# nosnoc/LCQPow

Hardware: AMD Instinct MI355X
Metric: LCQPs/sec (batched dense n=256,nC=512,nComp=64) (higher is better)
Workload: dtype f64; 1 GPU; synthetic dense batch=1024/GPU n=256 nC=512 nComp=64 (BASELINE configs[2]; SplitMix64 seed0=0x4C43515000000001, perturbStep=0, printLevel=NONE); global_batch=1024, parallelism=batch-sharded x1, no collective, solved=1024

## Files before the change

lcqpow_amd/csrc/lcqp_dev.hpp:

```cpp
#pragma once
#include "lcqp_wg.hpp"
#include "../../include/lcqp_hip.h"

namespace lcqp {

enum { V_G, V_GPHI, V_GTIL, V_XK, V_PK, V_XNEW, V_GK, V_QX, V_CX, V_QP, V_CP, V_STATK, V_TMP,
       V_XQ, V_XA, V_XT, V_R1, V_C, V_DU, V_W, V_RHS, V_LB, V_UB, V_X0, V_R1S, V_GS, V_ATY, V_QXN, V_XS, V_XREF, V_NUM };
enum { M_L, M_U, M_RHOV, M_YQ, M_YA, M_ZA, M_YT, M_EX, M_COEF, M_EXS, M_DY, M_RN, M_MG, M_YLV, M_HOTV, M_NUM };
enum { I_ST, I_STT, I_DEP, I_PRIO, I_SLOT, I_LIST, I_LIST2, I_HOTC, I_NUM };
enum { S_R2, S_DY, S_D0, S_SV, S_W, S_NUM };

struct InstInfo {
    int mE, nfin, hasY0, setupFail, haveSolution, isSetup, nT, prioCtr;
    int ndep, ns;
    int cNnz, kReady, rnReady, nHot;
    double scale, sigma, spv, rhoAdmm, phiConst;
    int warm, pad0;
    double rho0;
    double hist[64];
    double work[6];
};

struct DevBatch {
    int B, n, np, nC, nComp, mA, boxcap, mEcap, capS, nblk, nd;
// ... 19 lines not shown
};

template <int NCH>
struct Ctx {
    static constexpr int np = 128 * NCH;
    const DevBatch* db;
    int b, n, nC, nComp, mA, mE, capS, nblk;
    double *Q, *C, *E, *Et, *F1, *FK, *S, *S2, *DS, *D1, *dscr, *MM;
    double *nv, *mv, *sv;
    int *mi, *idx, *boxidx, *crow;
    InstInfo* info;
    Lds lds;
    int cAdmm, cTrials, cFact, cCorr, cSweeps;
#ifdef LCQP_PROFILE
    unsigned long long prof[16], tlast;
#endif

    __device__ __forceinline__ double* V(int k) const { return nv + (size_t)k * np; }
    __device__ __forceinline__ double* M(int k) const { return mv + (size_t)k * db->mEcap; }
    __device__ __forceinline__ int* I(int k) const { return mi + (size_t)k * db->mEcap; }
    __device__ __forceinline__ double* Sv(int k) const { return sv + (size_t)k * db->capS; }
};

template <int NCH>
__device__ __forceinline__ Ctx<NCH> make_ctx(const DevBatch& db, int b, Lds lds)
{
    Ctx<NCH> c;
    constexpr int np = 128 * NCH;
    c.db = &db; c.b = b; c.n = db.n; c.nC = db.nC; c.nComp = db.nComp; c.mA = db.mA; c.capS = db.capS; c.nblk = db.nblk;
    c.Q = db.Q + (size_t)b * np * np; c.C = db.C + (size_t)b * np * np;
    c.E = db.E + (size_t)b * db.mEcap * np; c.Et = db.Et + (size_t)b * db.mEcap * np;
    c.F1 = db.F1 + (size_t)b * np * np; c.FK = db.FK + (size_t)b * np * np;
    c.S = db.S + (size_t)b * db.capS * db.capS;
    c.MM = db.MM + (size_t)b * db.mMld * db.mMld;
    c.S2 = db.S2 + (size_t)b * db.capS * db.capS; c.DS = db.DS + (size_t)b * (db.capS / 64) * 4096;
    c.crow = db.crow + (size_t)b * db.capS;
    c.D1 = db.D1 + (size_t)b * db.nblk * 4096; c.dscr = db.dscr + (size_t)b * 4096;
    c.nv = db.nv + (size_t)b * V_NUM * np; c.mv = db.mv + (size_t)b * M_NUM * db.mEcap;
    c.sv = db.sv + (size_t)b * S_NUM * db.capS;
    c.mi = db.mi + (size_t)b * I_NUM * db.mEcap; c.idx = db.idx + (size_t)b * db.capS;
    c.boxidx = db.boxidx + (size_t)b * np;
    c.info = db.info + b;
    c.mE = uniform_i(c.info->mE);
    c.lds = lds;
    c.cAdmm = c.cTrials = c.cFact = c.cCorr = c.cSweeps = 0;
#ifdef LCQP_PROFILE
    for (int k = 0; k < 16; k++) c.prof[k] = 0;
    c.tlast = clock64();
#endif
    return c;
}

enum { P_LCQP = 0, P_RESID = 1, P_GRAM = 2, P_CHOL = 3, P_CORR_L1 = 4, P_CORR_ROWS = 5, P_CORR_S = 6, P_ADMM = 7, P_MISC = 8, P_DEL = 9, P_UPD_PRE = 10 };
#if defined(LCQP_PROFILE) && !defined(LCQP_PROFILE_BULK)
#define PROF(c, k) do { unsigned long long t_ = clock64(); (c).prof[k] += t_ - (c).tlast; (c).tlast = t_; } while (0)
#else
#define PROF(c, k) do { } while (0)
#endif
#if defined(LCQP_PROFILE) && defined(LCQP_PROFILE_BULK)
#define PROFB0(c) do { (c).tlast = clock64(); } while (0)
#define PROFB(c, k) do { unsigned long long t_ = clock64(); (c).prof[k] += t_ - (c).tlast; (c).tlast = t_; } while (0)
#else
#define PROFB0(c) do { } while (0)
#define PROFB(c, k) do { } while (0)
#endif

__device__ __forceinline__ double clipd(double v, double lo, double hi) { return v < lo ? lo : (v > hi ? hi : v); }

template <int NCH>
__device__ __forceinline__ void qp_admm(Ctx<NCH>& c, const double* g, int n_it)
{
    constexpr int np = 128 * NCH;
    const lcqp_options_t& o = c.db->opt;
    const int t = tid_here(), mE = c.mE;
    const double alpha = o.admmAlpha, sigma = c.info->sigma;
    double *xa = c.V(V_XA), *rhs = c.V(V_RHS), *w = c.V(V_W);
    double *ya = c.M(M_YA), *za = c.M(M_ZA), *rhov = c.M(M_RHOV), *coef = c.M(M_COEF), *ex = c.M(M_EX), *dyl = c.M(M_DY);
    const double *l = c.M(M_L), *u = c.M(M_U);
    PROF(c, P_MISC);
    for (int it = 0; it < n_it; it++) {
        const int t = tid_here();
        for (int r = t; r < mE; r += WG) coef[r] = rhov[r] * za[r] - ya[r];
        __syncthreads();
        wg_rows<NCH>(c.E, nullptr, mE, nullptr, nullptr, coef, c.lds,
                     [&](int i, double s) { rhs[i] = sigma * xa[i] - g[i] + s; });
        wg_trsv<wg_ncopy(NCH) == 2>(c.FK, np, c.nblk, rhs, true, c.lds);
        wg_trsv<wg_ncopy(NCH) == 2>(c.FK, np, c.nblk, rhs, false, c.lds);
        wg_rows<NCH>(c.E, nullptr, mE, rhs, ex, nullptr, c.lds, [](int, double) {});
        const bool last = (it == n_it - 1);
        for (int r = t; r < mE; r += WG) {
            const double zr = alpha * ex[r] + (1.0 - alpha) * za[r];
            const double rv = rhov[r];
            const double yold = ya[r];
            double yn;
            if (rv > 0.0) {
                const double zn = clipd(zr + yold / rv, l[r], u[r]);
                yn = yold + rv * (zr - zn);
                za[r] = zn;
            } else {
                za[r] = zr;
                yn = 0.0;
            }
            ya[r] = yn;
            if (last) dyl[r] = yn - yold;
        }
        for (int i = t; i < np; i += WG) {
            const double xold = xa[i], xn = alpha * rhs[i] + (1.0 - alpha) * xold;
            xa[i] = xn;
            if (last) w[i] = xn - xold;
        }
// ... 160 lines not shown
constexpr int TI_FAST_CHUNKS = 4;

template <int NCH>
__device__ __forceinline__ void ti_reset(Ctx<NCH>& c, int& nT, int& ns)
{
    int* rslot = c.I(I_SLOT);
    for (int r = tid_here(); r < c.mE; r += WG) rslot[r] = -1;
    for (int a = tid_here(); a < c.capS; a += WG) c.idx[a] = -1;
    nT = 0; ns = 0;
    __syncthreads();
}

template <int NK, int D>
__device__ __forceinline__ void ti_apply_fast(const double* __restrict__ Ti, int ld, const double* tv, double* out, int nT, int ns, double* red, const int* crow, const int* slotRow)
{
    const int l = lane_id(), w = wave_id(), t = tid_here();
    double tr[NK], acc[NK];
    int first[NK];
#pragma unroll
    for (int k = 0; k < NK; k++) {
        const int sl = 64 * k + l; tr[k] = (sl < ns) ? tv[sl] : 0.0; acc[k] = 0.0;
        first[k] = (sl < ns && slotRow[sl] >= 0) ? crow[sl] : (1 << 30);
    }
    for (int j0 = w; j0 < nT; j0 += NWAVE * D) {
        double rv[D][NK];
#pragma unroll
        for (int d = 0; d < D; d++) {
            const int j = j0 + NWAVE * d;
#pragma unroll
            for (int k = 0; k < NK; k++) {
                const int sl = 64 * k + l;
                rv[d][k] = (j < nT && j >= first[k]) ? Ti[(size_t)j * ld + sl] : 0.0;
            }
        }
#pragma unroll
        for (int d = 0; d < D; d++) {
            double dsum = 0.0;
#pragma unroll
            for (int k = 0; k < NK; k++) dsum += rv[d][k] * tr[k];
            const double u = wave_sum(dsum);
#pragma unroll
            for (int k = 0; k < NK; k++) acc[k] += rv[d][k] * u;
        }
    }
    __syncthreads();
#pragma unroll
    for (int k = 0; k < NK; k++) red[w * 256 + 64 * k + l] = acc[k];
    __syncthreads();
    for (int sl = t; sl < 64 * NK; sl += WG) out[sl] = (sl < ns) ? (red[sl] + red[256 + sl]) + (red[512 + sl] + red[768 + sl]) : 0.0;
    __syncthreads();
}

template <int NCH>
__device__ __forceinline__ void ti_apply(Ctx<NCH>& c, const double* tv, double* out, int nT, int ns)
{
    const int ld = c.capS, l = lane_id(), w = wave_id(), t = tid_here();
    const int nk = (ns + 63) >> 6;
    const double* Ti = c.S;
    if (nk <= TI_FAST_CHUNKS) {
        double* red = c.lds.arena;
        if (nk <= 1) ti_apply_fast<1, 16>(Ti, ld, tv, out, nT, ns, red, c.crow, c.idx);
        else if (nk == 2) ti_apply_fast<2, 8>(Ti, ld, tv, out, nT, ns, red, c.crow, c.idx);
        else if (nk == 3) ti_apply_fast<3, 6>(Ti, ld, tv, out, nT, ns, red, c.crow, c.idx);
        else ti_apply_fast<4, 4>(Ti, ld, tv, out, nT, ns, red, c.crow, c.idx);
    } else {
        constexpr int MAXK = (max_active(NCH) + 63) / 64;
        double* ts = c.lds.arena;
        double* us = c.lds.arena + 64 * nk;
        for (int sl = t; sl < 64 * nk; sl += WG) ts[sl] = (sl < ns) ? tv[sl] : 0.0;
        __syncthreads();
        for (int j = w; j < nT; j += NWAVE) {
            double dsum = 0.0;
#pragma unroll 4
            for (int k = 0; k < nk; k++) { const int sl = 64 * k + l; dsum += (sl < ns ? Ti[(size_t)j * ld + sl] : 0.0) * ts[sl]; }
            dsum = wave_sum(dsum);
            if (l == 0) us[j] = dsum;
        }
        __syncthreads();
        double acc[MAXK];
#pragma unroll
        for (int k = 0; k < MAXK; k++) acc[k] = 0.0;
        for (int j = w; j < nT; j += NWAVE) {
            const double u = us[j];
#pragma unroll
            for (int k = 0; k < MAXK; k++) { const int sl = 64 * k + l; if (k < nk && sl < ns) acc[k] += Ti[(size_t)j * ld + sl] * u; }
        }
        __syncthreads();
        double* red = c.lds.arena;
#pragma unroll
        for (int k = 0; k < MAXK; k++) if (k < nk) red[w * 64 * nk + 64 * k + l] = acc[k];
        __syncthreads();
        for (int sl = t; sl < 64 * nk; sl += WG)
            out[sl] = (sl < ns) ? (red[sl] + red[64 * nk + sl]) + (red[2 * 64 * nk + sl] + red[3 * 64 * nk + sl]) : 0.0;
        __syncthreads();
    }
}

template <int NCH>
__device__ __forceinline__ int ti_bulk(Ctx<NCH>& c, int na, double tau, int& nT, int& ns)
{
    const int ld = c.capS, t = tid_here(), mMld = c.db->mMld;
    const int nb = (na + 63) >> 6, nn = 64 * nb;
    int *idx = c.idx, *rslot = c.I(I_SLOT), *dep = c.I(I_DEP);
    double *F = c.S2, *Ti = c.S, *DS = c.DS;
    nT = na; ns = na;
    if (na == 0) return 0;
    PROFB0(c);
    {
        const int tot = nn * nn;
        int i = t / nn, j = t - i * nn;
        for (int e0 = t; e0 < tot; e0 += 8 * WG) {
            double v[8]; int ii[8], jj[8];
#pragma unroll
            for (int u = 0; u < 8; u++) {
                ii[u] = i; jj[u] = j;
                const bool in = (e0 + u * WG < tot) && (j <= i);
                v[u] = (i == j) ? 1.0 : 0.0;
                if (in && i < na) { const int ri = idx[i], rj = idx[j]; v[u] = c.MM[(size_t)max(ri, rj) * mMld + min(ri, rj)]; }
                if (!in) ii[u] = -1;
                j += WG; while (j >= nn) { j -= nn; i++; }
            }
#pragma unroll
            for (int u = 0; u < 8; u++) if (ii[u] >= 0) F[(size_t)ii[u] * ld + jj[u]] = v[u];
        }
    }
    __syncthreads();
    PROFB(c, 0);
    wg_chol(F, ld, nb, na, tau, DS, c.Sv(S_D0), nullptr, c.lds, 4096);
    PROFB(c, 1);
    {
        const int tot = nn * nn;
        int i = t / nn, j = t - i * nn;
        for (int e0 = t; e0 < tot; e0 += 8 * WG) {
            double v[8]; int ii[8], jj[8];
#pragma unroll
            for (int u = 0; u < 8; u++) {
                ii[u] = (e0 + u * WG < tot && (j >> 6) >= (i >> 6)) ? i : -1; jj[u] = j;
                v[u] = 0.0;
                if (ii[u] >= 0 && (i >> 6) == (j >> 6)) v[u] = DS[(size_t)(i >> 6) * 4096 + (i & 63) * 64 + (j & 63)];
                j += WG; while (j >= nn) { j -= nn; i++; }
            }
#pragma unroll
            for (int u = 0; u < 8; u++) if (ii[u] >= 0) Ti[(size_t)ii[u] * ld + jj[u]] = v[u];
        }
    }
    __syncthreads();
    PROFB(c, 2);
    auto ident = [](int r) { return (long)r; };
// ... 352 lines not shown
                    __syncthreads();
                } else
                if (res_stat <= rtolS && res_eq <= o.resTol * (1.0 + bmax)) {
                    double *r1s = c.V(V_R1S), *gs0 = c.V(V_GS), *exs = c.M(M_EXS), *aty = c.V(V_ATY);
                    double* qxn = c.V(V_QXN);
                    for (int i = t; i < np; i += WG) { const double ro = du[i]; r1s[i] = ro; gs0[i] = g[i]; aty[i] = g[i] + qx[i] + ro; qxn[i] = qx[i]; }
                    wg_map<4>(mE, [&](int r) { return ex[r]; }, [&](int r, double v) { exs[r] = v; });
                    __syncthreads();
                    PROF(c, P_RESID);
                    return 1;
                }
            }
            have_true = 1;
            PROF(c, P_RESID);
        }
        if (changed) fact_valid = 0;
        if (!fact_valid) {
            int nT = uniform_i(c.info->nT), ns = uniform_i(c.info->ns);
            int touched = 0, ndepNow = 0;
            const int ndel = wg_compact(ns, [&](int sl) { const int r = idx[sl]; return r >= 0 && st[r] == ST_INACT; }, list, c.lds);
            int cntAdd = 0;
            wg_map<4>(mE, [&](int r) { return MapID{st[r], (double)rslot[r]}; }, [&](int, MapID v) { cntAdd += (v.s != ST_INACT && v.a < 0.0); });
            const int nadd = block_sum_i(cntAdd, c.lds);
            if (trial >= 2 && nT - ndel + nadd > c.n && ndel + nadd > max(c.n / 2, 32)) return give_up();
            PROF(c, P_UPD_PRE);
            const bool bulk = (ROBUST && prioCtr > 0) || (nT == 0 && nadd > 0) || (ndel > 0 && ndel >= max(nT / 2, 8)) || nadd >= 16 || (3 * ndel + 7 * nadd >= 96);
            int naAll = 0;
            if (bulk) {
                int cntAct = 0;
                for (int r = t; r < mE; r += WG) cntAct += (st[r] != ST_INACT);
                naAll = block_sum_i(cntAct, c.lds);
                ti_reset<NCH>(c, nT, ns);
            }
            if (bulk && naAll <= capNa) {
                int na2 = 0;
                if (ROBUST)
                    for (int stamp = prioCtr; stamp >= 1; stamp--)
                        na2 += wg_compact(mE, [&](int r) { return st[r] != ST_INACT && prio[r] == stamp; }, idx + na2, c.lds);
                na2 += wg_compact(mE, [&](int r) { return st[r] != ST_INACT && (!ROBUST || prioCtr == 0 || prio[r] == 0); }, idx + na2, c.lds);
                if (LR) {
                    double *gyt = c.M(M_YT), *gex = c.M(M_EX), *gmg = c.M(M_MG); int* gst = c.I(I_STT);
                    for (int r = t; r < mE; r += WG) { gyt[r] = yt[r]; gex[r] = ex[r]; gmg[r] = mg[r]; gst[r] = st[r]; }
                    __syncthreads();
                }
                ndepNow = ti_bulk<NCH>(c, na2, o.depTau, nT, ns);
                if (LR) {
                    const double *gyt = c.M(M_YT), *gex = c.M(M_EX), *gmg = c.M(M_MG); const int* gst = c.I(I_STT);
                    __syncthreads();
                    for (int r = t; r < mE; r += WG) { yt[r] = gyt[r]; ex[r] = gex[r]; mg[r] = gmg[r]; st[r] = gst[r]; }
                    __syncthreads();
                }
                touched = 1;
                PROF(c, P_GRAM);
#ifdef LCQP_PROFILE
                c.prof[11] += 1; c.prof[12] += (unsigned long long)na2;
#endif
            } else {
                if (!bulk)
                    for (int k = 0; k < ndel; k++) {
                        const int sl = uniform_i(list[k]);
                        ti_delete<NCH>(c, sl, nT, ns);
                        touched = 1;
                    }
                PROF(c, P_DEL);
#ifdef LCQP_PROFILE
                if (!bulk) c.prof[13] += (unsigned long long)ndel;
#endif
                for (int stamp = (ROBUST && bulk) ? prioCtr : 0; stamp >= 0; stamp--) {
                    const int cnt = wg_compact(mE, [&](int r) { return st[r] != ST_INACT && rslot[r] < 0 && (stamp == 0 || prio[r] == stamp); }, list, c.lds);
                    for (int k = 0; k < cnt; k++) {
                        const int r = uniform_i(list[k]);
                        const int rc = ti_append<NCH>(c, r, o.depTau, capNa, nT, ns);
                        if (rc < 0) { if (t == 0) { c.info->nT = nT; c.info->ns = ns; } __syncthreads(); return give_up(); }
                        if (ROBUST && t == 0) dep[r] = (rc == 0);
                        ndepNow += (rc == 0);
                        touched = 1;
#ifdef LCQP_PROFILE
                        c.prof[14] += 1;
#endif
                    }
                }
            }
            if (ROBUST) {
                if (ndepNow > 0 || uniform_i(c.info->ndep) > 0) {
                    __syncthreads();
                    for (int r = t; r < mE; r += WG) if (st[r] == ST_INACT || rslot[r] >= 0) dep[r] = 0;
                }
                if (t == 0) c.info->ndep = ndepNow;
            }
            PROF(c, P_CHOL);
            na = nT; nsl = ns;
            if (touched) { c.cFact++; if (t == 0) c.info->work[3] += 1.0; }
            if (t == 0) { c.info->nT = nT; c.info->ns = ns; }
            __syncthreads();
            fact_valid = 1;
        }
        const int nsp = 64 * ((nsl + 63) >> 6);
#ifdef LCQP_TRACE_QP
        if (tid_here() == 0) printf("  hip trial %d damp %d: left %d changed %d true %d na %d ns %d dep %d\n", trial, damp, nlv, changed, have_true, na, nsl, ROBUST ? c.info->ndep : 0);
#endif
        if (have_true) {
            for (int a = t; a < nsp; a += WG) {
                double v = 0.0;
                const int r = (a < nsl) ? idx[a] : -1;
                if (r >= 0) { const double bb = (st[r] == ST_UPPER) ? u[r] : l[r]; v = bb - ex[r]; }
                r2[a] = v;
            }
            wg_copy(cv, r1, np);
            PROF(c, P_MISC);
            wg_trsv<wg_ncopy(NCH) == 2>(c.F1, np, c.nblk, cv, true, c.lds);
            PROF(c, P_CORR_L1);
            if (na > 0) {
                wg_rows<NCH, false, true>(c.Et, idx, nsl, cv, dy, nullptr, c.lds, [](int, double) {});
                for (int a = t; a < nsp; a += WG) dy[a] = (a < nsl && idx[a] >= 0) ? dy[a] - r2[a] : 0.0;
                __syncthreads();
                PROF(c, P_CORR_ROWS);
            }
            if (t == 0) { c.info->work[0] += 2.0 * na; c.info->work[5] += 2.0; }
        } else {
            int nl = 0;
            if (nlv > 0) {
                nl = wg_compact(mE, [&](int r) { return ylv[r] != 0.0; }, list, c.lds);
                wg_rows<NCH, true>(c.Et, list, nl, nullptr, nullptr, ylv, c.lds, [&](int i, double s) { cv[i] = s; });
            }
            const int mMld = c.db->mMld;
            for (int a = t; a < nsp; a += WG) {
                double v = 0.0;
                const int r = (a < nsl) ? idx[a] : -1;
                if (r >= 0) {
                    const double bb = (st[r] == ST_UPPER) ? u[r] : l[r];
                    for (int k = 0; k < nl; k++) { const int rl = list[k]; v += ylv[rl] * c.MM[(size_t)max(rl, r) * mMld + min(rl, r)]; }
                    v -= bb - ex[r];
                }
                dy[a] = v;
            }
            __syncthreads();
            for (int k = t; k < nl; k += WG) ylv[list[k]] = 0.0;
            if (t == 0) { c.info->work[0] += (double)(na + nl); c.info->work[5] += 1.0; c.info->work[2] += 8.0 * (double)nl * nsl; }
            nlv = nl;
            PROF(c, P_CORR_ROWS);
        }
        if (na > 0) {
            ti_apply<NCH>(c, dy, dy, na, nsl);
            PROF(c, P_CORR_S);
            const bool withC = have_true || nlv > 0;
            wg_rows<NCH>(c.Et, idx, nsl, nullptr, nullptr, dy, c.lds, [&](int i, double s) { du[i] = (withC ? cv[i] : 0.0) - s; });
            PROF(c, P_CORR_ROWS);
        } else {
            if (have_true || nlv > 0) wg_copy(du, cv, np);
            else wg_fill(du, 0.0, np);
        }
        wg_trsv<wg_ncopy(NCH) == 2>(c.F1, np, c.nblk, du, false, c.lds);
        PROF(c, P_CORR_L1);
        for (int i = t; i < np; i += WG) x[i] += du[i];
        for (int a = t; a < nsl; a += WG) {
            const int r = idx[a];
            if (r >= 0) { yt[r] += dy[a]; ex[r] = (st[r] == ST_UPPER) ? u[r] : l[r]; }
        }
        if (t == 0) c.info->work[1] += (nsl <= 64 * TI_FAST_CHUNKS) ? 0.5 * (double)na * (na + 1) : (double)na * nsl;
        __syncthreads();
        c.cCorr++;
    }
    return give_up();
}

template <int NCH, bool ROBUST, bool ADAPT, bool LR = false>
__device__ __forceinline__ int qp_solve(Ctx<NCH>& c, int initial, const double* g, const double* y0ref, int* iterations, double gmaxHint = -1.0, int checkBounds = 1)
{
    constexpr int np = 128 * NCH;
    const lcqp_options_t& o = c.db->opt;
    const int t = tid_here(), mE = c.mE, n = c.n, nC = c.mA;
    const int trials0 = c.cTrials, admm0 = c.cAdmm;
    *iterations = 0;
    if (uniform_i(c.info->setupFail)) return 3;
    double *xq = c.V(V_XQ), *xa = c.V(V_XA), *xt = c.V(V_XT);
    double *yq = c.M(M_YQ), *ya = c.M(M_YA), *za = c.M(M_ZA), *ex = c.M(M_EX);
    double* yt = LR ? c.lds.arena + LDS_ROWS_OFF : c.M(M_YT);
    int* stt = LR ? reinterpret_cast<int*>(c.lds.arena + LDS_ROWS_OFF + 3 * LDS_ROWS_MAX) : c.I(I_STT);
    const double *l = c.M(M_L), *u = c.M(M_U), *rhov = c.M(M_RHOV);
    int* st = c.I(I_ST);
    if (checkBounds) {
        int bad = 0;
        wg_map<4>(mE, [&](int r) { return MapD4{l[r], u[r], 0.0, 0.0}; }, [&](int, MapD4 v) { bad |= (v.a > v.b); });
        if (block_or(bad, c.lds)) return 2;
    }
    const double gsc = uniform_d(1.0 + (gmaxHint >= 0.0 ? gmaxHint : wg_maxabs(g, c.n, c.lds)));
    const double ytolQ = uniform_d(o.feasTol * gsc), rtolQ = uniform_d(o.resTol * gsc);
    if (ROBUST && uniform_i(c.info->prioCtr) != 0) {
        int* prio = c.I(I_PRIO);
        for (int r = t; r < mE; r += WG) prio[r] = 0;
        __syncthreads();
        if (t == 0) c.info->prioCtr = 0;
        __syncthreads();
    }
    if (initial) {
        const double* x0 = c.V(V_X0);
        for (int i = t; i < np; i += WG) xq[i] = x0[i];
        for (int r = t; r < mE; r += WG) {
            double yr = 0.0;
            if (y0ref) yr = (r < nC) ? -y0ref[n + r] : -y0ref[c.boxidx[r - nC]];
            yq[r] = yr;
        }
        __syncthreads();
    }
    for (int i = t; i < np; i += WG) { const double v = xq[i]; xa[i] = v; c.V(V_XREF)[i] = v; }
    wg_map<4>(mE, [&](int r) { return yq[r]; }, [&](int r, double v) { ya[r] = v; });
    __syncthreads();
    int n_admm = initial ? o.admmFirst : o.admmHot;
    const int haveSol = uniform_i(c.info->haveSolution);
    const int use_stored = (!initial && haveSol && n_admm == 0);
    int reuse_stored = use_stored && haveSol != 2;
    if (ROBUST && use_stored && uniform_i(c.info->ndep) > 0) {
        const int* dep = c.I(I_DEP);
// ... 328 lines not shown
```

lcqpow_amd/csrc/lcqp_wg.hpp:

```cpp
#pragma once
#include <hip/hip_runtime.h>
#include <stdint.h>

namespace lcqp {

constexpr int WG = 256;
constexpr int NWAVE = 4;
constexpr int wg_ncopy(int nch) { return nch > 16 ? 2 : 4; }
constexpr int arena_doubles(int nch) { return (wg_ncopy(nch) + 2) * 128 * nch > 4512 ? (wg_ncopy(nch) + 2) * 128 * nch : 4512; }
constexpr int ARENA = arena_doubles(4);
constexpr int TILE_LD = 65;
constexpr int max_active(int nch) { return 64 * (arena_doubles(nch) / (5 * 64)); }
constexpr int LCQP_MAX_ACTIVE = max_active(4);

enum { ST_INACT = 0, ST_LOWER = 1, ST_UPPER = 2, ST_EQ = 3 };

constexpr int LDS_ROWS_MAX = 640;
constexpr int LDS_ROWS_OFF = 2048;
static_assert(LDS_ROWS_OFF + 3 * LDS_ROWS_MAX + LDS_ROWS_MAX / 2 <= 4512, "row state must fit the arena");

struct Lds {
    double* arena;
    double* red;
    int* ired;
};
#define LCQP_LDS_N(NCHV)                                    \
    __shared__ double sh_arena[arena_doubles(NCHV)];        \
    __shared__ double sh_red[16];                           \
    __shared__ int sh_ired[16];                             \
    Lds lds{sh_arena, sh_red, sh_ired};
#define LCQP_LDS LCQP_LDS_N(4)

typedef double d2v_t __attribute__((ext_vector_type(2)));
__device__ __forceinline__ double2 ld_stream(const double2* p) { const d2v_t v = __builtin_nontemporal_load(reinterpret_cast<const d2v_t*>(p)); return double2{v.x, v.y}; }
__device__ __forceinline__ double ld_stream(const double* p) { return __builtin_nontemporal_load(p); }

__device__ __forceinline__ int tid_here() { int t = threadIdx.x; asm volatile("" : "+v"(t)); return t; }
__device__ __forceinline__ int lane_id() { return tid_here() & 63; }
__device__ __forceinline__ int wave_id() { return tid_here() >> 6; }

__device__ __forceinline__ double wave_sum(double v)
{
#pragma unroll
    for (int o = 32; o > 0; o >>= 1) v += __shfl_xor(v, o, 64);
    return v;
}
__device__ __forceinline__ double wave_max(double v)
{
#pragma unroll
    for (int o = 32; o > 0; o >>= 1) v = fmax(v, __shfl_xor(v, o, 64));
    return v;
}
__device__ __forceinline__ double wave_bcast(double v, int src)
{
    const int lo = __builtin_amdgcn_readlane(__double2loint(v), src);
    const int hi = __builtin_amdgcn_readlane(__double2hiint(v), src);
    return __hiloint2double(hi, lo);
}
__device__ __forceinline__ int wave_bcast_i(int v, int src) { return __builtin_amdgcn_readlane(v, src); }
__device__ __forceinline__ int wave_sum_i(int v)
{
#pragma unroll
    for (int o = 32; o > 0; o >>= 1) v += __shfl_xor(v, o, 64);
    return v;
}

__device__ __forceinline__ double uniform_d(double v)
{
    const int lo = __builtin_amdgcn_readfirstlane(__double2loint(v));
    const int hi = __builtin_amdgcn_readfirstlane(__double2hiint(v));
    return __hiloint2double(hi, lo);
}
// ... 225 lines not shown
    if (TWO_M && o10) wg_combine<NCH>(a10, lds, [&](int c, double s) { o10[c] = s; });
    if (TWO_V && o01) wg_combine<NCH>(a01, lds, [&](int c, double s) { o01[c] = s; });
    if (TWO_M && TWO_V && o11) wg_combine<NCH>(a11, lds, [&](int c, double s) { o11[c] = s; });
}

template <int NCH>
__device__ __forceinline__ void wg_symv(const double* __restrict__ M0, const double* __restrict__ M1, int n,
                        const double* __restrict__ v0, const double* __restrict__ v1,
                        double* o00, double* o10, double* o01, double* o11, Lds lds)
{
    if (M1 != nullptr && v1 != nullptr) wg_symv_t<NCH, true, true>(M0, M1, n, v0, v1, o00, o10, o01, o11, lds);
    else if (M1 != nullptr) wg_symv_t<NCH, true, false>(M0, M1, n, v0, nullptr, o00, o10, nullptr, nullptr, lds);
    else if (v1 != nullptr) wg_symv_t<NCH, false, true>(M0, nullptr, n, v0, v1, o00, nullptr, o01, nullptr, lds);
    else wg_symv_t<NCH, false, false>(M0, nullptr, n, v0, nullptr, o00, nullptr, nullptr, nullptr, lds);
}

template <int NCH>
__device__ __forceinline__ void wg_row_norms(const double* __restrict__ Mx, int m, double* out, int* hotc = nullptr, double* hotv = nullptr)
{
    constexpr int np = 128 * NCH;
    const int l = lane_id(), w = wave_id();
    for (int r0 = w; r0 < m; r0 += 4 * NWAVE) {
        double2 mm[4][NCH];
#pragma unroll
        for (int d = 0; d < 4; d++) {
            const int r = r0 + NWAVE * d;
#pragma unroll
            for (int k = 0; k < NCH; k++) mm[d][k] = (r < m) ? (reinterpret_cast<const double2*>(Mx + (size_t)r * np) + l)[64 * k] : double2{0.0, 0.0};
        }
#pragma unroll
        for (int d = 0; d < 4; d++) {
            double s2 = 0.0;
#pragma unroll
            for (int k = 0; k < NCH; k++) s2 += mm[d][k].x * mm[d][k].x + mm[d][k].y * mm[d][k].y;
            s2 = wave_sum(s2);
            const int r = r0 + NWAVE * d;
            if (l == 0 && r < m) out[r] = sqrt(s2);
            if (hotc && r < m) {
                int cnt = 0, col = -1; double val = 0.0;
#pragma unroll
                for (int k = 0; k < NCH; k++) {
                    if (mm[d][k].x != 0.0) { cnt++; col = 128 * k + 2 * l; val = mm[d][k].x; }
                    if (mm[d][k].y != 0.0) { cnt++; col = 128 * k + 2 * l + 1; val = mm[d][k].y; }
                }
                const int tot = wave_sum_i(cnt);
                if (tot == 1) { if (cnt == 1) { hotc[r] = col; hotv[r] = val; } }
                else if (l == 0) hotc[r] = -1;
            }
        }
    }
    __syncthreads();
}

template <int NCH, bool BYROW = false, bool KEEP = false, class Post>
__device__ __forceinline__ void wg_rows(const double* __restrict__ Mx, const int* __restrict__ idx, int m,
                        const double* __restrict__ x, double* dots,
                        const double* __restrict__ coef, Lds lds, Post post,
                        const int* __restrict__ hotc = nullptr, const double* __restrict__ hotv = nullptr)
{
    constexpr int np = 128 * NCH;
    static_assert((wg_ncopy(NCH) + 1) * np <= arena_doubles(NCH), "wg_rows: the partial copies and the staged vector must fit the LDS arena");
    double* sx = lds.arena + wg_ncopy(NCH) * np;
    if (x) {
        for (int i = tid_here(); i < np; i += WG) sx[i] = x[i];
    }
    __syncthreads();
    const int l = lane_id(), w = wave_id();
    double xr[2 * NCH], acc[2 * NCH];
#pragma unroll
    for (int k = 0; k < NCH; k++) {
        xr[2 * k] = x ? sx[128 * k + 2 * l] : 0.0;
        xr[2 * k + 1] = x ? sx[128 * k + 2 * l + 1] : 0.0;
        acc[2 * k] = acc[2 * k + 1] = 0.0;
    }
    const int nchunk = (m + 15) >> 4;
    constexpr int D = (NCH > 8) ? 1 : (NCH == 4 ? 2 : ROWS_IN_FLIGHT);
    for (int ch = w; ch < nchunk; ch += NWAVE) {
        const int a0 = ch << 4;
        const int mya = a0 + l;
        const bool mine = (l < 16) && (mya < m);
        int myrow = mine ? (idx ? idx[mya] : mya) : -1;
        double mycoef = (mine && coef && (!BYROW || myrow >= 0)) ? coef[BYROW ? myrow : mya] : 0.0;
        const int myhc = (hotc && myrow >= 0) ? hotc[myrow] : -1;
        const double myhv = (myhc >= 0) ? hotv[myrow] : 0.0;
        double mydot = 0.0;
        const int cnt = min(16, m - a0);
        for (int j0 = 0; j0 < cnt; j0 += D) {
            double2 mm[D][NCH];
            int rows[D];
            double cfs[D];
#pragma unroll
            for (int d = 0; d < D; d++) {
                rows[d] = wave_bcast_i(myrow, (j0 + d) & 63);
                cfs[d] = wave_bcast(mycoef, (j0 + d) & 63);
                const int hc = hotc ? wave_bcast_i(myhc, (j0 + d) & 63) : -1;
                if (hc >= 0) {
                    const double hv = wave_bcast(myhv, (j0 + d) & 63);
#pragma unroll
                    for (int k = 0; k < NCH; k++) {
                        mm[d][k] = double2{0.0, 0.0};
                        if ((hc >> 7) == k && ((hc & 127) >> 1) == l) { if (hc & 1) mm[d][k].y = hv; else mm[d][k].x = hv; }
                    }
                } else if (rows[d] >= 0) {
                    const double2* rp = reinterpret_cast<const double2*>(Mx + (size_t)rows[d] * np) + l;
#pragma unroll
                    for (int k = 0; k < NCH; k++) mm[d][k] = KEEP ? rp[64 * k] : ld_stream(rp + 64 * k);
                } else {
#pragma unroll
                    for (int k = 0; k < NCH; k++) mm[d][k] = double2{0.0, 0.0};
                }
            }
#pragma unroll
            for (int d = 0; d < D; d++) {
                if (x) {
                    double dsum = 0.0;
#pragma unroll
                    for (int k = 0; k < NCH; k++) dsum += mm[d][k].x * xr[2 * k] + mm[d][k].y * xr[2 * k + 1];
                    dsum = wave_sum(dsum);
                    if (l == j0 + d) mydot = dsum;
                }
                if (coef && cfs[d] != 0.0) {
#pragma unroll
                    for (int k = 0; k < NCH; k++) { acc[2 * k] += cfs[d] * mm[d][k].x; acc[2 * k + 1] += cfs[d] * mm[d][k].y; }
                }
            }
        }
        if (mine && dots && (!BYROW || myrow >= 0)) dots[BYROW ? myrow : mya] = mydot;
    }
    if (coef) wg_combine<NCH>(acc, lds, post);
    else __syncthreads();
}

template <bool TWO = false>
__device__ __forceinline__ void wg_trsv(const double* __restrict__ F, int ld, int nblk, double* vec, bool forward, Lds lds)
{
    const int nn = 64 * nblk;
    double* b = lds.arena;
    double* red = lds.arena + nn;
    for (int i = tid_here(); i < nn; i += WG) b[i] = vec[i];
    __syncthreads();
    const int l = lane_id(), w = wave_id();
    for (int s = 0; s < nblk; s++) {
        const int I = forward ? s : nblk - 1 - s;
        {
            const double* Fd = F + (size_t)(64 * I) * ld + 64 * I;
            double f[16];
#pragma unroll
            for (int cc = 0; cc < 16; cc++) {
                const int c = 16 * w + cc;
                f[cc] = 0.0;
                if (forward ? (c <= l) : (c >= l)) f[cc] = ld_stream(Fd + (size_t)c * ld + l);
            }
            double acc = 0.0;
#pragma unroll
            for (int cc = 0; cc < 16; cc++) {
                const int c = 16 * w + cc;
                const bool use = forward ? (c <= l) : (c >= l);
                acc += use ? f[cc] * b[64 * I + c] : 0.0;
            }
            red[w * 64 + l] = acc;
        }
        __syncthreads();
        if (tid_here() < 64) b[64 * I + tid_here()] = red[l] + red[64 + l] + red[128 + l] + red[192 + l];
        __syncthreads();
        const int cb0 = forward ? I + 1 : 0, cb1 = forward ? nblk : I;
        if (cb1 > cb0) {
            constexpr bool two = TWO;
            for (int pass = 0; pass < (two ? 2 : 1); pass++) {
                if (!two || (w >> 1) == pass)
                    for (int cb = cb0; cb < cb1; cb++) {
                        const double* Fp = F + (size_t)(64 * I + 16 * w) * ld + 64 * cb + l;
                        double f[16];
#pragma unroll
                        for (int cc = 0; cc < 16; cc++) f[cc] = ld_stream(Fp + (size_t)cc * ld);
                        double acc = 0.0;
#pragma unroll
                        for (int cc = 0; cc < 16; cc++) acc += f[cc] * b[64 * I + 16 * w + cc];
                        if (!two) red[w * nn + 64 * cb + l] = acc;
                        else if (pass == 0) red[(w & 1) * nn + 64 * cb + l] = acc;
                        else red[(w & 1) * nn + 64 * cb + l] += acc;
                    }
                __syncthreads();
            }
            for (int c = 64 * cb0 + tid_here(); c < 64 * cb1; c += WG)
                b[c] -= two ? (red[c] + red[nn + c]) : (red[c] + red[nn + c] + red[2 * nn + c] + red[3 * nn + c]);
            __syncthreads();
        }
    }
    for (int i = tid_here(); i < nn; i += WG) vec[i] = b[i];
    __syncthreads();
}

constexpr int TILE_PL = 80;
typedef double d4_t __attribute__((ext_vector_type(4)));

__device__ __forceinline__ int tile_li(int a, int b)
{
    (void)a; return 16 * wave_id() + (lane_id() >> 4) + 4 * b;
}
__device__ __forceinline__ int tile_lj(int a, int b)
{
    (void)b; return 16 * a + (lane_id() & 15);
}

__device__ __forceinline__ void tile_panel(double (&acc)[4][4], const double* As, const double* Bs)
{
    const int il = lane_id() & 15, kl = lane_id() >> 4, w = wave_id();
    d4_t c[4];
#pragma unroll
    for (int a = 0; a < 4; a++) c[a] = d4_t{acc[a][0], acc[a][1], acc[a][2], acc[a][3]};
#pragma unroll
    for (int k4 = 0; k4 < 4; k4++) {
        const double av = As[(4 * k4 + kl) * TILE_PL + 16 * w + il];
#pragma unroll
        for (int a = 0; a < 4; a++) {
            const double bv = Bs[(4 * k4 + kl) * TILE_PL + 16 * a + il];
            c[a] = __builtin_amdgcn_mfma_f64_16x16x4f64(av, bv, c[a], 0, 0, 0);
        }
    }
#pragma unroll
    for (int a = 0; a < 4; a++) { acc[a][0] = c[a][0]; acc[a][1] = c[a][1]; acc[a][2] = c[a][2]; acc[a][3] = c[a][3]; }
}

template <class RowA, class RowB>
__device__ __forceinline__ void wg_tile_nt(double (&acc)[4][4], const double* __restrict__ A, int lda, RowA rowA,
                                           const double* __restrict__ Bm, int ldb, RowB rowB, int K, Lds lds,
                                           int rowsValid = 64)
{
    const bool active = 16 * wave_id() < rowsValid;
    constexpr int PL = TILE_PL;
    double* As = lds.arena;
    double* Bs = lds.arena + 16 * PL;
    const int t = tid_here();
    const int lr = t >> 2, kq = (t & 3) * 4;
    const long ra = rowA(lr), rb = rowB(lr);
    const double* ap = (ra >= 0) ? A + (size_t)ra * lda + kq : nullptr;
    const double* bp = (rb >= 0) ? Bm + (size_t)rb * ldb + kq : nullptr;
#pragma unroll
    for (int i = 0; i < 4; i++)
#pragma unroll
        for (int j = 0; j < 4; j++) acc[i][j] = 0.0;
    double2 a0 = {0.0, 0.0}, a1 = {0.0, 0.0}, b0 = {0.0, 0.0}, b1 = {0.0, 0.0};
    if (ap && K > 0) { a0 = *reinterpret_cast<const double2*>(ap); a1 = *reinterpret_cast<const double2*>(ap + 2); }
// ... 262 lines not shown
```

Before: 31100 LCQPs/s.

## Keep correction-step chain vectors in LDS and fuse staging across trsv and row kernels

For NCH<=2, the corrector chain now keeps the intermediate vectors (c, dy, the staged x) in the LDS arena between the forward triangular solve, the row dot products, the T-inverse apply and the backward solve. Callbacks replace the global-memory round trips. Generic wg_rows_io and wg_trsv_io variants take lambdas for input and output, so the per-step global copies, the r2 buffer and several barriers go away. It also adds an optional chain profiling mode. The costs are tighter LDS layout constraints and more code paths, with a fallback through global memory when the active set is wide.

```diff
diff --git a/lcqpow_amd/csrc/lcqp_dev.hpp b/lcqpow_amd/csrc/lcqp_dev.hpp
--- a/lcqpow_amd/csrc/lcqp_dev.hpp
+++ b/lcqpow_amd/csrc/lcqp_dev.hpp
@@ -95,10 +95,19 @@
 }
 
 enum { P_LCQP = 0, P_RESID = 1, P_GRAM = 2, P_CHOL = 3, P_CORR_L1 = 4, P_CORR_ROWS = 5, P_CORR_S = 6, P_ADMM = 7, P_MISC = 8, P_DEL = 9, P_UPD_PRE = 10 };
+#if defined(LCQP_PROFILE) && defined(LCQP_PROFILE_CHAIN)
+enum { PC_R2 = 0, PC_COPY = 1, PC_L1F = 2, PC_ROWS1 = 3, PC_SUBR2 = 4, PC_T = 5, PC_ROWS2 = 6, PC_L1B = 7, PC_UPD = 8, PC_REST = 9, PC_PRED = 10 };
+#define PROFC(c, k) do { unsigned long long t_ = clock64(); (c).prof[k] += t_ - (c).tlast; (c).tlast = t_; } while (0)
+#define PROFC_COUNT(c, k) do { (c).prof[k] += 1; } while (0)
+#define PROF(c, k) PROFC(c, PC_REST)
+#else
+#define PROFC(c, k) do { } while (0)
+#define PROFC_COUNT(c, k) do { } while (0)
 #if defined(LCQP_PROFILE) && !defined(LCQP_PROFILE_BULK)
 #define PROF(c, k) do { unsigned long long t_ = clock64(); (c).prof[k] += t_ - (c).tlast; (c).tlast = t_; } while (0)
 #else
 #define PROF(c, k) do { } while (0)
+#endif
 #endif
 #if defined(LCQP_PROFILE) && defined(LCQP_PROFILE_BULK)
 #define PROFB0(c) do { (c).tlast = clock64(); } while (0)
@@ -365,18 +374,26 @@
 }
 
 template <int NCH>
-__device__ __forceinline__ void ti_apply(Ctx<NCH>& c, const double* tv, double* out, int nT, int ns)
-{
-    const int ld = c.capS, l = lane_id(), w = wave_id(), t = tid_here();
+__device__ __forceinline__ void ti_apply_narrow(Ctx<NCH>& c, const double* tv, double* out, int nT, int ns)
+{
+    const int ld = c.capS;
     const int nk = (ns + 63) >> 6;
     const double* Ti = c.S;
-    if (nk <= TI_FAST_CHUNKS) {
+    {
         double* red = c.lds.arena;
         if (nk <= 1) ti_apply_fast<1, 16>(Ti, ld, tv, out, nT, ns, red, c.crow, c.idx);
         else if (nk == 2) ti_apply_fast<2, 8>(Ti, ld, tv, out, nT, ns, red, c.crow, c.idx);
         else if (nk == 3) ti_apply_fast<3, 6>(Ti, ld, tv, out, nT, ns, red, c.crow, c.idx);
         else ti_apply_fast<4, 4>(Ti, ld, tv, out, nT, ns, red, c.crow, c.idx);
-    } else {
+    }
+}
+template <int NCH>
+__device__ __forceinline__ void ti_apply_wide(Ctx<NCH>& c, const double* tv, double* out, int nT, int ns)
+{
+    const int ld = c.capS, l = lane_id(), w = wave_id(), t = tid_here();
+    const int nk = (ns + 63) >> 6;
+    const double* Ti = c.S;
+    {
         constexpr int MAXK = (max_active(NCH) + 63) / 64;
         double* ts = c.lds.arena;
         double* us = c.lds.arena + 64 * nk;
@@ -407,6 +424,12 @@
             out[sl] = (sl < ns) ? (red[sl] + red[64 * nk + sl]) + (red[2 * 64 * nk + sl] + red[3 * 64 * nk + sl]) : 0.0;
         __syncthreads();
     }
+}
+template <int NCH>
+__device__ __forceinline__ void ti_apply(Ctx<NCH>& c, const double* tv, double* out, int nT, int ns)
+{
+    if (((ns + 63) >> 6) <= TI_FAST_CHUNKS) ti_apply_narrow<NCH>(c, tv, out, nT, ns);
+    else ti_apply_wide<NCH>(c, tv, out, nT, ns);
 }
 
 template <int NCH>
@@ -865,7 +888,7 @@
                 }
                 touched = 1;
                 PROF(c, P_GRAM);
-#ifdef LCQP_PROFILE
+#if defined(LCQP_PROFILE) && !defined(LCQP_PROFILE_CHAIN)
                 c.prof[11] += 1; c.prof[12] += (unsigned long long)na2;
 #endif
             } else {
@@ -876,7 +899,7 @@
                         touched = 1;
                     }
                 PROF(c, P_DEL);
-#ifdef LCQP_PROFILE
+#if defined(LCQP_PROFILE) && !defined(LCQP_PROFILE_CHAIN)
                 if (!bulk) c.prof[13] += (unsigned long long)ndel;
 #endif
                 for (int stamp = (ROBUST && bulk) ? prioCtr : 0; stamp >= 0; stamp--) {
@@ -888,7 +911,7 @@
                         if (ROBUST && t == 0) dep[r] = (rc == 0);
                         ndepNow += (rc == 0);
                         touched = 1;
-#ifdef LCQP_PROFILE
+#if defined(LCQP_PROFILE) && !defined(LCQP_PROFILE_CHAIN)
                         c.prof[14] += 1;
 #endif
                     }
@@ -912,66 +935,166 @@
 #ifdef LCQP_TRACE_QP
         if (tid_here() == 0) printf("  hip trial %d damp %d: left %d changed %d true %d na %d ns %d dep %d\n", trial, damp, nlv, changed, have_true, na, nsl, ROBUST ? c.info->ndep : 0);
 #endif
-        if (have_true) {
-            for (int a = t; a < nsp; a += WG) {
-                double v = 0.0;
-                const int r = (a < nsl) ? idx[a] : -1;
-                if (r >= 0) { const double bb = (st[r] == ST_UPPER) ? u[r] : l[r]; v = bb - ex[r]; }
-                r2[a] = v;
-            }
-            wg_copy(cv, r1, np);
-            PROF(c, P_MISC);
-            wg_trsv<wg_ncopy(NCH) == 2>(c.F1, np, c.nblk, cv, true, c.lds);
+        PROFC(c, PC_REST);
+        PROFC_COUNT(c, 14);
+        if constexpr (NCH <= 2) {
+            double* lb = c.lds.arena;
+            double* sx = wg_rows_x(c.lds, np);
+            double* lcv = c.lds.arena + LDS_CHAIN_C_OFF;
+            double* ldy = c.lds.arena + LDS_CHAIN_DY_OFF;
+            auto bound_of = [&](int r) -> double { return (st[r] == ST_UPPER) ? u[r] : l[r]; };
+            if (have_true) {
+                PROFC_COUNT(c, 11);
+                PROF(c, P_MISC);
+                wg_trsv_io(c.F1, np, c.nblk, [&](int i) { return r1[i]; }, [&](int i, double v) { sx[i] = v; lcv[i] = v; }, true, c.lds);
+                PROFC(c, PC_L1F);
+                PROF(c, P_CORR_L1);
+                if (na > 0) {
+                    wg_rows_io<NCH, true, true>(c.Et, idx, nsl, nullptr, true, false, [](int, int) { return 0.0; },
+                                                [&](int a, int r, double d) { ldy[a] = (r >= 0) ? d - (bound_of(r) - ex[r]) : 0.0; },
+                                                c.lds, [](int, double) {});
+                    PROFC(c, PC_ROWS1);
+                    PROF(c, P_CORR_ROWS);
+                }
+                if (t == 0) { c.info->work[0] += 2.0 * na; c.info->work[5] += 2.0; }
+            } else {
+                PROFC_COUNT(c, 12);
+                int nl = 0;
+                if (nlv > 0) {
+                    nl = wg_compact(mE, [&](int r) { return ylv[r] != 0.0; }, list, c.lds);
+                    wg_rows<NCH, true>(c.Et, list, nl, nullptr, nullptr, ylv, c.lds, [&](int i, double s) { lcv[i] = s; });
+                }
+                const int mMld = c.db->mMld;
+                for (int a = t; a < nsp; a += WG) {
+                    double v = 0.0;
+                    const int r = (a < nsl) ? idx[a] : -1;
+                    if (r >= 0) {
+                        const double bb = bound_of(r);
+                        for (int k = 0; k < nl; k++) { const int rl = list[k]; v += ylv[rl] * c.MM[(size_t)max(rl, r) * mMld + min(rl, r)]; }
+                        v -= bb - ex[r];
+                    }
+                    ldy[a] = v;
+                }
+                __syncthreads();
+                for (int k = t; k < nl; k += WG) ylv[list[k]] = 0.0;
+                if (t == 0) { c.info->work[0] += (double)(na + nl); c.info->work[5] += 1.0; c.info->work[2] += 8.0 * (double)nl * nsl; }
+                nlv = nl;
+                PROFC(c, PC_PRED);
+                PROF(c, P_CORR_ROWS);
+            }
+            if (na > 0) {
+                if (nsp <= 64 * TI_FAST_CHUNKS) {
+                    ti_apply_narrow<NCH>(c, ldy, ldy, na, nsl);
+                } else {
+                    for (int i = t; i < np; i += WG) cv[i] = lcv[i];
+                    for (int a = t; a < nsp; a += WG) dy[a] = (a < nsl) ? ldy[a] : 0.0;
+                    __syncthreads();
+                    ti_apply_wide<NCH>(c, dy, dy, na, nsl);
+                    for (int i = t; i < np; i += WG) lcv[i] = cv[i];
+                    for (int a = t; a < nsp; a += WG) ldy[a] = dy[a];
+                    __syncthreads();
+                }
+                PROFC(c, PC_T);
+                PROF(c, P_CORR_S);
+                for (int a = t; a < nsl; a += WG) {
+                    const int r = idx[a];
+                    if (r >= 0) { yt[r] += ldy[a]; ex[r] = bound_of(r); }
+                }
+                PROFC(c, PC_UPD);
+                const bool withC = have_true || nlv > 0;
+                wg_rows_io<NCH, false, true>(c.Et, idx, nsl, nullptr, false, true, [&](int a, int) { return ldy[a]; }, [](int, int, double) {},
+                                             c.lds, [&](int i, double s) { lb[i] = (withC ? lcv[i] : 0.0) - s; });
+                PROFC(c, PC_ROWS2);
+                PROF(c, P_CORR_ROWS);
+            } else {
+                PROFC_COUNT(c, 13);
+                if (!have_true) {
+                    const bool withC = nlv > 0;
+                    for (int i = t; i < np; i += WG) lb[i] = withC ? lcv[i] : 0.0;
+                    __syncthreads();
+                }
+                PROFC(c, PC_COPY);
+            }
+            wg_trsv_io<false, true>(c.F1, np, c.nblk, [](int) { return 0.0; }, [&](int i, double v) { x[i] += v; }, false, c.lds);
+            PROFC(c, PC_L1B);
             PROF(c, P_CORR_L1);
+            if (t == 0) c.info->work[1] += (nsl <= 64 * TI_FAST_CHUNKS) ? 0.5 * (double)na * (na + 1) : (double)na * nsl;
+        } else {
+            if (have_true) {
+                PROFC_COUNT(c, 11);
+                for (int a = t; a < nsp; a += WG) {
+                    double v = 0.0;
+                    const int r = (a < nsl) ? idx[a] : -1;
+                    if (r >= 0) { const double bb = (st[r] == ST_UPPER) ? u[r] : l[r]; v = bb - ex[r]; }
+                    r2[a] = v;
+                }
+                PROFC(c, PC_R2);
+                wg_copy(cv, r1, np);
+                PROFC(c, PC_COPY);
+                PROF(c, P_MISC);
+                wg_trsv<wg_ncopy(NCH) == 2>(c.F1, np, c.nblk, cv, true, c.lds);
+                PROFC(c, PC_L1F);
+                PROF(c, P_CORR_L1);
+                if (na > 0) {
+                    wg_rows<NCH, false, true>(c.Et, idx, nsl, cv, dy, nullptr, c.lds, [](int, double) {});
+                    PROFC(c, PC_ROWS1);
+                    for (int a = t; a < nsp; a += WG) dy[a] = (a < nsl && idx[a] >= 0) ? dy[a] - r2[a] : 0.0;
+                    __syncthreads();
+                    PROFC(c, PC_SUBR2);
+                    PROF(c, P_CORR_ROWS);
+                }
+                if (t == 0) { c.info->work[0] += 2.0 * na; c.info->work[5] += 2.0; }
+            } else {
+                PROFC_COUNT(c, 12);
+                int nl = 0;
+                if (nlv > 0) {
+                    nl = wg_compact(mE, [&](int r) { return ylv[r] != 0.0; }, list, c.lds);
+                    wg_rows<NCH, true>(c.Et, list, nl, nullptr, nullptr, ylv, c.lds, [&](int i, double s) { cv[i] = s; });
+                }
+                const int mMld = c.db->mMld;
+                for (int a = t; a < nsp; a += WG) {
+                    double v = 0.0;
+                    const int r = (a < nsl) ? idx[a] : -1;
+                    if (r >= 0) {
+                        const double bb = (st[r] == ST_UPPER) ? u[r] : l[r];
+                        for (int k = 0; k < nl; k++) { const int rl = list[k]; v += ylv[rl] * c.MM[(size_t)max(rl, r) * mMld + min(rl, r)]; }
+                        v -= bb - ex[r];
+                    }
+                    dy[a] = v;
+                }
+                __syncthreads();
+                for (int k = t; k < nl; k += WG) ylv[list[k]] = 0.0;
+                if (t == 0) { c.info->work[0] += (double)(na + nl); c.info->work[5] += 1.0; c.info->work[2] += 8.0 * (double)nl * nsl; }
+                nlv = nl;
+                PROFC(c, PC_PRED);
+                PROF(c, P_CORR_ROWS);
+            }
             if (na > 0) {
-                wg_rows<NCH, false, true>(c.Et, idx, nsl, cv, dy, nullptr, c.lds, [](int, double) {});
-                for (int a = t; a < nsp; a += WG) dy[a] = (a < nsl && idx[a] >= 0) ? dy[a] - r2[a] : 0.0;
-                __syncthreads();
+                ti_apply<NCH>(c, dy, dy, na, nsl);
+                PROFC(c, PC_T);
+                PROF(c, P_CORR_S);
+                const bool withC = have_true || nlv > 0;
+                wg_rows<NCH>(c.Et, idx, nsl, nullptr, nullptr, dy, c.lds, [&](int i, double s) { du[i] = (withC ? cv[i] : 0.0) - s; });
+                PROFC(c, PC_ROWS2);
                 PROF(c, P_CORR_ROWS);
-            }
-            if (t == 0) { c.info->work[0] += 2.0 * na; c.info->work[5] += 2.0; }
-        } else {
-            int nl = 0;
-            if (nlv > 0) {
-                nl = wg_compact(mE, [&](int r) { return ylv[r] != 0.0; }, list, c.lds);
-                wg_rows<NCH, true>(c.Et, list, nl, nullptr, nullptr, ylv, c.lds, [&](int i, double s) { cv[i] = s; });
-            }
-            const int mMld = c.db->mMld;
-            for (int a = t; a < nsp; a += WG) {
-                double v = 0.0;
-                const int r = (a < nsl) ? idx[a] : -1;
-                if (r >= 0) {
-                    const double bb = (st[r] == ST_UPPER) ? u[r] : l[r];
-                    for (int k = 0; k < nl; k++) { const int rl = list[k]; v += ylv[rl] * c.MM[(size_t)max(rl, r) * mMld + min(rl, r)]; }
-                    v -= bb - ex[r];
-                }
-                dy[a] = v;
-            }
+            } else {
+                PROFC_COUNT(c, 13);
+                if (have_true || nlv > 0) wg_copy(du, cv, np);
+                else wg_fill(du, 0.0, np);
+                PROFC(c, PC_COPY);
+            }
+            wg_trsv<wg_ncopy(NCH) == 2>(c.F1, np, c.nblk, du, false, c.lds);
+            PROFC(c, PC_L1B);
+            PROF(c, P_CORR_L1);
+            for (int i = t; i < np; i += WG) x[i] += du[i];
+            for (int a = t; a < nsl; a += WG) {
+                const int r = idx[a];
+                if (r >= 0) { yt[r] += dy[a]; ex[r] = (st[r] == ST_UPPER) ? u[r] : l[r]; }
+            }
+            if (t == 0) c.info->work[1] += (nsl <= 64 * TI_FAST_CHUNKS) ? 0.5 * (double)na * (na + 1) : (double)na * nsl;
             __syncthreads();
-            for (int k = t; k < nl; k += WG) ylv[list[k]] = 0.0;
-            if (t == 0) { c.info->work[0] += (double)(na + nl); c.info->work[5] += 1.0; c.info->work[2] += 8.0 * (double)nl * nsl; }
-            nlv = nl;
-            PROF(c, P_CORR_ROWS);
-        }
-        if (na > 0) {
-            ti_apply<NCH>(c, dy, dy, na, nsl);
-            PROF(c, P_CORR_S);
-            const bool withC = have_true || nlv > 0;
-            wg_rows<NCH>(c.Et, idx, nsl, nullptr, nullptr, dy, c.lds, [&](int i, double s) { du[i] = (withC ? cv[i] : 0.0) - s; });
-            PROF(c, P_CORR_ROWS);
-        } else {
-            if (have_true || nlv > 0) wg_copy(du, cv, np);
-            else wg_fill(du, 0.0, np);
-        }
-        wg_trsv<wg_ncopy(NCH) == 2>(c.F1, np, c.nblk, du, false, c.lds);
-        PROF(c, P_CORR_L1);
-        for (int i = t; i < np; i += WG) x[i] += du[i];
-        for (int a = t; a < nsl; a += WG) {
-            const int r = idx[a];
-            if (r >= 0) { yt[r] += dy[a]; ex[r] = (st[r] == ST_UPPER) ? u[r] : l[r]; }
-        }
-        if (t == 0) c.info->work[1] += (nsl <= 64 * TI_FAST_CHUNKS) ? 0.5 * (double)na * (na + 1) : (double)na * nsl;
-        __syncthreads();
+            PROFC(c, PC_UPD);
+        }
         c.cCorr++;
     }
     return give_up();
diff --git a/lcqpow_amd/csrc/lcqp_wg.hpp b/lcqpow_amd/csrc/lcqp_wg.hpp
--- a/lcqpow_amd/csrc/lcqp_wg.hpp
+++ b/lcqpow_amd/csrc/lcqp_wg.hpp
@@ -18,6 +18,11 @@
 constexpr int LDS_ROWS_MAX = 640;
 constexpr int LDS_ROWS_OFF = 2048;
 static_assert(LDS_ROWS_OFF + 3 * LDS_ROWS_MAX + LDS_ROWS_MAX / 2 <= 4512, "row state must fit the arena");
+
+constexpr int LDS_CHAIN_C_OFF = 1280;
+constexpr int LDS_CHAIN_DY_OFF = LDS_CHAIN_C_OFF + 256;
+static_assert(LDS_CHAIN_DY_OFF + LDS_ROWS_OFF / 4 <= LDS_ROWS_OFF, "chain vectors must end below the row state");
+static_assert(LDS_CHAIN_DY_OFF + LCQP_MAX_ACTIVE <= ARENA, "chain vectors must fit the arena");
 
 struct Lds {
     double* arena;
@@ -349,25 +354,28 @@
     __syncthreads();
 }
 
-template <int NCH, bool BYROW = false, bool KEEP = false, class Post>
-__device__ __forceinline__ void wg_rows(const double* __restrict__ Mx, const int* __restrict__ idx, int m,
-                        const double* __restrict__ x, double* dots,
-                        const double* __restrict__ coef, Lds lds, Post post,
+__device__ __forceinline__ double* wg_rows_x(Lds lds, int np) { return lds.arena + 4 * np; }
+template <int NCH, bool KEEP = false, bool STAGED = false, class Coef, class Dot, class Post>
+__device__ __forceinline__ void wg_rows_io(const double* __restrict__ Mx, const int* __restrict__ idx, int m,
+                        const double* __restrict__ x, bool hasx, bool hascoef, Coef coeff, Dot dotf, Lds lds, Post post,
                         const int* __restrict__ hotc = nullptr, const double* __restrict__ hotv = nullptr)
 {
     constexpr int np = 128 * NCH;
     static_assert((wg_ncopy(NCH) + 1) * np <= arena_doubles(NCH), "wg_rows: the partial copies and the staged vector must fit the LDS arena");
+    static_assert(!STAGED || wg_ncopy(NCH) == 4, "wg_rows_io: wg_rows_x assumes four partial copies");
     double* sx = lds.arena + wg_ncopy(NCH) * np;
-    if (x) {
-        for (int i = tid_here(); i < np; i += WG) sx[i] = x[i];
-    }
-    __syncthreads();
+    if (!STAGED) {
+        if (hasx) {
+            for (int i = tid_here(); i < np; i += WG) sx[i] = x[i];
+        }
+        __syncthreads();
+    }
     const int l = lane_id(), w = wave_id();
     double xr[2 * NCH], acc[2 * NCH];
 #pragma unroll
     for (int k = 0; k < NCH; k++) {
-        xr[2 * k] = x ? sx[128 * k + 2 * l] : 0.0;
-        xr[2 * k + 1] = x ? sx[128 * k + 2 * l + 1] : 0.0;
+        xr[2 * k] = hasx ? sx[128 * k + 2 * l] : 0.0;
+        xr[2 * k + 1] = hasx ? sx[128 * k + 2 * l + 1] : 0.0;
         acc[2 * k] = acc[2 * k + 1] = 0.0;
     }
     const int nchunk = (m + 15) >> 4;
@@ -377,7 +385,7 @@
         const int mya = a0 + l;
         const bool mine = (l < 16) && (mya < m);
         int myrow = mine ? (idx ? idx[mya] : mya) : -1;
-        double mycoef = (mine && coef && (!BYROW || myrow >= 0)) ? coef[BYROW ? myrow : mya] : 0.0;
+        double mycoef = (mine && hascoef) ? coeff(mya, myrow) : 0.0;
         const int myhc = (hotc && myrow >= 0) ? hotc[myrow] : -1;
         const double myhv = (myhc >= 0) ? hotv[myrow] : 0.0;
         double mydot = 0.0;
@@ -409,33 +417,47 @@
             }
 #pragma unroll
             for (int d = 0; d < D; d++) {
-                if (x) {
+                if (hasx) {
                     double dsum = 0.0;
 #pragma unroll
                     for (int k = 0; k < NCH; k++) dsum += mm[d][k].x * xr[2 * k] + mm[d][k].y * xr[2 * k + 1];
                     dsum = wave_sum(dsum);
                     if (l == j0 + d) mydot = dsum;
                 }
-                if (coef && cfs[d] != 0.0) {
+                if (hascoef && cfs[d] != 0.0) {
 #pragma unroll
                     for (int k = 0; k < NCH; k++) { acc[2 * k] += cfs[d] * mm[d][k].x; acc[2 * k + 1] += cfs[d] * mm[d][k].y; }
                 }
             }
         }
-        if (mine && dots && (!BYROW || myrow >= 0)) dots[BYROW ? myrow : mya] = mydot;
-    }
-    if (coef) wg_combine<NCH>(acc, lds, post);
+        if (mine && hasx) dotf(mya, myrow, mydot);
+    }
+    if (hascoef) wg_combine<NCH>(acc, lds, post);
     else __syncthreads();
 }
 
-template <bool TWO = false>
-__device__ __forceinline__ void wg_trsv(const double* __restrict__ F, int ld, int nblk, double* vec, bool forward, Lds lds)
+template <int NCH, bool BYROW = false, bool KEEP = false, class Post>
+__device__ __forceinline__ void wg_rows(const double* __restrict__ Mx, const int* __restrict__ idx, int m,
+                        const double* __restrict__ x, double* dots,
+                        const double* __restrict__ coef, Lds lds, Post post,
+                        const int* __restrict__ hotc = nullptr, const double* __restrict__ hotv = nullptr)
+{
+    wg_rows_io<NCH, KEEP>(Mx, idx, m, x, x != nullptr, coef != nullptr,
+                          [&](int a, int row) { return (!BYROW || row >= 0) ? coef[BYROW ? row : a] : 0.0; },
+                          [&](int a, int row, double d) { if (dots && (!BYROW || row >= 0)) dots[BYROW ? row : a] = d; },
+                          lds, post, hotc, hotv);
+}
+
+template <bool TWO = false, bool STAGED = false, class In, class Out>
+__device__ __forceinline__ void wg_trsv_io(const double* __restrict__ F, int ld, int nblk, In in, Out out, bool forward, Lds lds)
 {
     const int nn = 64 * nblk;
     double* b = lds.arena;
     double* red = lds.arena + nn;
-    for (int i = tid_here(); i < nn; i += WG) b[i] = vec[i];
-    __syncthreads();
+    if (!STAGED) {
+        for (int i = tid_here(); i < nn; i += WG) b[i] = in(i);
+        __syncthreads();
+    }
     const int l = lane_id(), w = wave_id();
     for (int s = 0; s < nblk; s++) {
         const int I = forward ? s : nblk - 1 - s;
@@ -484,8 +506,13 @@
             __syncthreads();
         }
     }
-    for (int i = tid_here(); i < nn; i += WG) vec[i] = b[i];
-    __syncthreads();
+    for (int i = tid_here(); i < nn; i += WG) out(i, b[i]);
+    __syncthreads();
+}
+template <bool TWO = false>
+__device__ __forceinline__ void wg_trsv(const double* __restrict__ F, int ld, int nblk, double* vec, bool forward, Lds lds)
+{
+    wg_trsv_io<TWO>(F, ld, nblk, [&](int i) { return vec[i]; }, [&](int i, double v) { vec[i] = v; }, forward, lds);
 }
 
 constexpr int TILE_PL = 80;
```

Result: no change. 31260 LCQPs/s (median of 6 runs) (+0.5%).
